# tobifinn/torch-assimilate

Measured on AMD Instinct MI355X. Metric: local analyses/sec (LETKF, 40-member), higher is better.
Workload: dtype f32

## Files before the change

### torch-assimilate_amd/csrc/letkf_tile2_kernel.h

```cpp
#pragma once
#include <type_traits>
#include "mia_common.h"
#include <hip/hip_ext.h>
#include "mia_kernels.h"
#include "mia_options.h"
#include "mia_tiles.h"
#ifdef MIA_TILE_STAMPS
namespace mia { constexpr int kT2StampN = 20, kT2StampTiles = 8192; static __device__ long long g_tile2_stamps[kT2StampTiles * kT2StampN]; }
#define MIA_TL_STAMP(i) do { if (lane == 0 && tile < mia::kT2StampTiles) mia::g_tile2_stamps[tile * mia::kT2StampN + 12 + (i)] = (long long)__builtin_amdgcn_s_memtime(); } while (0)
#endif
#include "mia_tile_localize.h"

namespace mia {

#ifdef MIA_TILE_STAMPS
#define T2_STAMP(i) do { if (lane == 0 && bid < kT2StampTiles) g_tile2_stamps[bid * kT2StampN + (i)] = (long long)__builtin_amdgcn_s_memtime(); } while (0)
#define T2_STAMP_HWID() do { if (lane == 0 && bid < kT2StampTiles) g_tile2_stamps[bid * kT2StampN + 9] = \
    (long long)(unsigned)__builtin_amdgcn_s_getreg((31 << 11) | 4) | ((long long)(unsigned)__builtin_amdgcn_s_getreg((31 << 11) | 20) << 32); } while (0)
#define T2_STAMP_REAL(i) do { if (lane == 0 && bid < kT2StampTiles) g_tile2_stamps[bid * kT2StampN + (i)] = (long long)__builtin_amdgcn_s_memrealtime(); } while (0)
#else
#define T2_STAMP(i) do { } while (0)
#define T2_STAMP_HWID() do { } while (0)
#define T2_STAMP_REAL(i) do { } while (0)
#endif

#ifndef MIA_TILE2_WAVES_UT2
#define MIA_TILE2_WAVES_UT2 4
#endif

template <int UT, int KT, bool MROWS, int LOC>
__device__ __forceinline__ void tile2_body(Tile2Params P, const Tile2Loc* loc, const int64_t bid) {
  constexpr int UMAX = 16 * UT, NB = (KT + 1) / 2, NKB = (UT + 1) / 2;
  extern __shared__ __attribute__((aligned(16))) unsigned char smem[];
  int lane = threadIdx.x, lr = lane & 15, h = lane >> 4;
  const int k = P.k, nc8 = P.nc8;
  const unsigned IMG = (unsigned)(UT * nc8) * 512u;
  unsigned char* zline = smem + IMG;
  int* ukey = reinterpret_cast<int*>(smem + IMG + 512);
  float* wdl = reinterpret_cast<float*>(ukey + UMAX);
  float* El = wdl + UMAX;

  const int64_t ntile = (P.ng + 15) >> 4;
  if (bid >= ntile) return;
  if (P.clr_counts) {
    const int ncl = *P.clr_n;
    for (int64_t i = bid * 64 + lane; i < ncl; i += ntile * 64) P.clr_counts[i] = 0;
    if (bid == 0 && lane == 0) {
      const unsigned e = *P.clr_err;
      if (e) { atomicOr(P.err_out, (int)(e << 3)); *P.clr_err = 0u; }
    }
  }
  const int64_t q8 = ntile >> 3, r8 = ntile & 7, xcd = bid & 7;
  const int64_t tile = (xcd < r8 ? xcd * (q8 + 1) : r8 * (q8 + 1) + (xcd - r8) * q8) + (bid >> 3);
  const int64_t p0 = tile << 4;
  const int npts = P.ng - p0 < 16 ? (int)(P.ng - p0) : 16;
  int64_t oc0 = P.o0 + p0;
  if (P.seg_len > 0) {
    const unsigned sgi = (unsigned)p0 / (unsigned)P.seg_len;
    oc0 = p0 - (int64_t)sgi * P.seg_len;
    P.Xa += (int64_t)sgi * P.seg_stride;
  }
  const unsigned ldxb = (unsigned)P.ldx * 4u, ldob = (unsigned)P.ldo * 4u;
  int lrc = lr < npts ? lr : npts - 1;
  bool colok = lr < npts;

#ifdef MIA_EXPERIMENTS
  const int prio_mode = (P.stagger >> 8) & 0xff, exp_trim = P.stagger >> 16;
  P.stagger &= 0xff;
  if (prio_mode == 1) __builtin_amdgcn_s_setprio(3);
  if (prio_mode >= 3) {
    const int wid = (int)(__builtin_amdgcn_s_getreg((4 << 11) | 4) & 0xf);
    const bool fast = prio_mode == 3 ? (wid & 1) : (prio_mode == 4 ? wid < 2 : (prio_mode == 5 ? wid == 0 : (wid % 3) == 0));
    if (fast) __builtin_amdgcn_s_setprio(3);
  }
  if (P.stagger > 0) {
    const int slot = (int)(__builtin_amdgcn_s_getreg((4 << 11) | 4) & 0xf);
    for (int i = 0; i < slot * P.stagger; ++i) __builtin_amdgcn_s_sleep(1);
  }
#endif
  T2_STAMP(0);
  T2_STAMP_HWID();
  T2_STAMP_REAL(10);
  int hdU = 0;
  int myidx[(UMAX + 63) / 64];
  f4w dreg[UT];
  if constexpr (LOC == 0) {
    const int4 hd = P.thdr[tile];
    hdU = hd.x;
#pragma unroll
    for (int r = 0; r < (UMAX + 63) / 64; ++r) {
      const int s = lane + 64 * r;
      myidx[r] = s < UMAX ? t2_ld<int32_t>(P.tidx + tile * UMAX, (unsigned)s * 4u) : -1;
    }
#pragma unroll
    for (int t = 0; t < UT; ++t) dreg[t] = t2_ld<f4w>(P.tD + (tile * UT + t) * 64, (unsigned)lane * 16u);
  } else {
    const TileLocOut lo = tile_localize<true, (LOC > 3 ? LOC - 4 : LOC), MIA_TAPER_GC, (LOC > 3)>(loc->scan, P.g0, P.ng, UT, tile, smem, lane);
    const TileLocLds LL(smem);
    hdU = lo.overflow ? -1 : lo.U;
    int mu[(UMAX + 63) / 64], du[UT][4];
#pragma unroll
    for (int r = 0; r < (UMAX + 63) / 64; ++r) {
      const int s = lane + 64 * r;
      mu[r] = LL.uinv[s < UMAX ? s : 0];
      mu[r] = (s < UMAX && !lo.overflow && mu[r] >= 0) ? mu[r] : kTlUmax;
    }
#pragma unroll
    for (int t = 0; t < UT; ++t)
#pragma unroll
      for (int qq = 0; qq < 4; ++qq) {
        du[t][qq] = LL.uinv[16 * t + 4 * h + qq];
        du[t][qq] = (!lo.overflow && du[t][qq] >= 0) ? du[t][qq] * 16 + lr : LL.zrow_off + lr;
      }
#pragma unroll
    for (int r = 0; r < (UMAX + 63) / 64; ++r) myidx[r] = LL.ukey[mu[r]];
#pragma unroll
    for (int t = 0; t < UT; ++t) {
      f4w v;
#pragma unroll
      for (int qq = 0; qq < 4; ++qq) v[qq] = LL.Wt[du[t][qq]];
      dreg[t] = v;
    }
    if (lane == 0) {
      if (lo.longest > loc->longest_bound) atomicMax(&loc->stats[0], lo.longest);
      else if ((tile & 63) == 0 && lo.longest > __hip_atomic_load(&loc->stats[0], __ATOMIC_RELAXED, __HIP_MEMORY_SCOPE_AGENT))
        atomicMax(&loc->stats[0], lo.longest);
      if (tile == 0) atomicOr(&loc->stats[3], kStepSampledLongest);
      if (lo.overflow) atomicAdd(&loc->stats[1], 1);
      if (lo.box_overflow) atomicOr(&loc->stats[1], MIA_TILE_BOX_OVERFLOW);
    }
    MIA_T2_SYNC();
  }
  int sg = 2 * (h & 1) + (h >> 1);
  auto load_xs = [&](int mi, float (&xr)[NB][8]) {
    const float* xbase = P.X + (int64_t)mi * k * P.ldx + P.g0 + p0;
#pragma unroll
    for (int b = 0; b < NB; ++b) {
      const int m0 = 8 * (4 * b + sg);
      if (b < NB - 1 || (k & 7) == 0) {
        const unsigned vo = (unsigned)(m0 < k ? m0 : 0) * ldxb + (unsigned)lrc * 4u;
#pragma unroll
        for (int i = 0; i < 8; ++i) xr[b][i] = t2_ld<float>(xbase, vo + (unsigned)i * ldxb);
      } else {
#pragma unroll
        for (int i = 0; i < 8; ++i) {
          const int mem = m0 + i;
          xr[b][i] = t2_ld<float>(xbase, (unsigned)(mem < k ? mem : k - 1) * ldxb + (unsigned)lrc * 4u);
        }
      }
    }
  };
  float xsb[NB][8];
  load_xs(0, xsb);
#pragma unroll
  for (int r = 0; r < (UMAX + 63) / 64; ++r) {
    const int s = lane + 64 * r;
    if (s < UMAX) ukey[s] = myidx[r];
  }
  for (int i = lane; i < 32; i += 64) reinterpret_cast<f4w*>(zline)[i] = f4w{0.f, 0.f, 0.f, 0.f};
  MIA_T2_SYNC();
  const int U = __builtin_amdgcn_readfirstlane(hdU);
  if (U < 0) {
    if (colok && h == 0) P.flags[p0 + lr] = MIA_FLAG_OVERFLOW;
    const float nanv = __builtin_nanf("");
    if (colok)
      for (int it = h; it < P.m * k; it += 4) P.Xa[(int64_t)it * P.ldo + oc0 + lr] = nanv;
    return;
  }
  T2_STAMP(1);
  {
    const int g = lane >> 4, hl = g & 1, gh = g >> 1;
    unsigned roff[UT][2];
#pragma unroll
    for (int t = 0; t < UT; ++t)
#pragma unroll
      for (int par = 0; par < 2; ++par) {
        const int idx = ukey[16 * t + ((lr - 8 * par) & 15)];
        roff[t][par] = (unsigned)(idx < 0 ? (int)P.zero_rec : idx) * (unsigned)P.rb + 16u * (unsigned)hl;
      }
    auto gather = [&](auto nc8c) {
      constexpr int NC8 = decltype(nc8c)::value;
      constexpr int NL = (UT * NC8 + 1) / 2;
#pragma unroll
      for (int u = 0; u < NL; ++u) {
        const int lA = 2 * u, lB = 2 * u + 1;
        const int tA = lA / NC8, cA = lA % NC8, tB = (lB / NC8) < UT ? lB / NC8 : UT - 1, cB = lB % NC8;
        const unsigned offA = roff[tA][cA & 1] + 32u * (unsigned)cA, offB = roff[tB][cB & 1] + 32u * (unsigned)cB;
        const unsigned off = gh ? offB : offA;
        const bool valid = 2 * u + gh < UT * NC8;
        if (valid)
          __builtin_amdgcn_global_load_lds(reinterpret_cast<const unsigned*>(P.rec + off),
                                           (__attribute__((address_space(3))) void*)(smem + u * 1024), 16, 0, 0);
      }
    };
    if (nc8 == 2 * KT - 1) gather(std::integral_constant<int, 2 * KT - 1>{});
    else gather(std::integral_constant<int, 2 * KT>{});
  }
  f2w tails[(UMAX + 63) / 64];
#pragma unroll
  for (int r = 0; r < (UMAX + 63) / 64; ++r) {
    const unsigned j = (unsigned)(myidx[r] < 0 ? (int)P.zero_rec : myidx[r]);
    tails[r] = *reinterpret_cast<const f2w*>(P.rec + (j * (unsigned)P.rb + 32u * (unsigned)nc8));
  }
  T2_STAMP(2);

  auto frag_off = [&](int t, int b) -> unsigned {
    const int c = 4 * b + sg;
    const unsigned col = (unsigned)((lr + 8 * (c & 1)) & 15) * 16u;
    return c < nc8 ? (unsigned)(t * nc8 + c) * 512u + col : IMG + col;
  };

  h8v GAh[UT][NKB], GAl[UT][NKB];
  float alpha = 0.0f;
  int deg = 0, tab_idx = 0, degmax = 0, pflag = 0;
  bool decl = false;
  auto split_x = [&](float (&xsb)[NB][8], float& xm, float& inv_sx, h8v (&xh)[NB], h8v (&xl)[NB]) {
      t2_split_x<NB, MROWS>(xsb, colok, sg, k, P.inv_k, xm, inv_sx, xh, xl);
    };
  float xm0, inv_sx0;
  f4w Z0[UT];
  {
    h8v xh[NB], xl[NB];
    split_x(xsb, xm0, inv_sx0, xh, xl);
#pragma unroll
    for (int t = 0; t < UT; ++t) Z0[t] = f4w{0.f, 0.f, 0.f, 0.f};
    f4w (&Z)[UT] = Z0;
    asm volatile("s_waitcnt vmcnt(0)" ::: "memory");
    __builtin_amdgcn_wave_barrier();
    T2_STAMP(3);
#ifdef MIA_EXPERIMENTS
    if (prio_mode == 1) __builtin_amdgcn_s_setprio(0);
    if (prio_mode == 2) __builtin_amdgcn_s_setprio(3);
#endif
    f4w G[UT][UT];
#pragma unroll
    for (int t1 = 0; t1 < UT; ++t1)
#pragma unroll
      for (int t2 = 0; t2 < UT; ++t2) G[t1][t2] = f4w{0.f, 0.f, 0.f, 0.f};
#pragma unroll
    for (int b = 0; b < NB; ++b) {
      h8v ah[UT], al[UT];
#pragma unroll
      for (int t = 0; t < UT; ++t) {
        const unsigned o = frag_off(t, b);
        ah[t] = *reinterpret_cast<const h8v*>(smem + o);
        al[t] = *reinterpret_cast<const h8v*>(smem + o + 256);
      }
#pragma unroll
      for (int t2 = 0; t2 < UT; ++t2)
#pragma unroll
        for (int t1 = 0; t1 < UT; ++t1) G[t1][t2] = t2_mfma3(G[t1][t2], ah[t1], al[t1], ah[t2], al[t2]);
#pragma unroll
      for (int t = 0; t < UT; ++t) Z[t] = t2_mfma3(Z[t], ah[t], al[t], xh[b], xl[b]);
    }
    T2_STAMP(4);
    {
      bool badrec = false;
#pragma unroll
      for (int r = 0; r < (UMAX + 63) / 64; ++r) {
        const int s = lane + 64 * r;
        if (s < UMAX) {
          wdl[s] = tails[r][0];
          El[s] = tails[r][1];
          badrec = badrec || !(tails[r][1] == tails[r][1]);
        }
      }
      if (__any(badrec)) {
        if (colok && h == 0) { P.flags[p0 + lr] = MIA_FLAG_RETRY; atomicAdd(P.retry_count, 1); }
        return;
      }
      MIA_T2_SYNC();
#pragma unroll
      for (int t = 0; t < UT; ++t) {
        const f4w e4 = *reinterpret_cast<const f4w*>(El + 16 * t + 4 * h);
        dreg[t] *= e4;
      }
    }
#pragma unroll
    for (int t = 0; t < UT; ++t)
#pragma unroll
      for (int kb = 0; kb < NKB; ++kb) {
        float gv[8];
#pragma unroll
        for (int tt = 0; tt < 2; ++tt)
#pragma unroll
          for (int q = 0; q < 4; ++q) gv[4 * tt + q] = 2 * kb + tt < UT ? G[2 * kb + tt < UT ? 2 * kb + tt : 0][t][q] * 0x1p-16f : 0.0f;
        split8(gv, GAh[t][kb], GAl[t][kb]);
      }
    f4w R[UT];
#pragma unroll
    for (int t = 0; t < UT; ++t) R[t] = f4w{0.f, 0.f, 0.f, 0.f};
    unsigned dmx = 0u;
#pragma unroll
    for (int t = 0; t < UT; ++t)
#pragma unroll
      for (int q = 0; q < 4; ++q) { const unsigned a = __float_as_uint(dreg[t][q]); dmx = a > dmx ? a : dmx; }
    dmx = t2_wave_max_u32(dmx);
    int esd;
    const float sd = pow2_scale(dmx, 0, &esd);
    const float inv_sd = __uint_as_float((unsigned)(127 - esd) << 23);
#pragma unroll
    for (int kb = 0; kb < NKB; ++kb)
      if (kb == 0 || 32 * kb < U) {
        float dv[8];
#pragma unroll
        for (int tt = 0; tt < 2; ++tt)
#pragma unroll
          for (int q = 0; q < 4; ++q) dv[4 * tt + q] = 2 * kb + tt < UT ? dreg[2 * kb + tt < UT ? 2 * kb + tt : 0][q] * sd : 0.0f;
        const h8v dh = hi8(dv);
#pragma unroll
        for (int t = 0; t < UT; ++t) {
          u4w ag = __builtin_bit_cast(u4w, GAh[t][kb]);
          ag &= 0x7fff7fffu;
          R[t] = __builtin_amdgcn_mfma_f32_16x16x32_f16(__builtin_bit_cast(h8v, ag), dh, R[t], 0, 0, 0);
        }
      }
    float L = 0.0f;
#pragma unroll
    for (int t = 0; t < UT; ++t)
#pragma unroll
      for (int q = 0; q < 4; ++q) L = __builtin_fmaxf(L, dreg[t][q] * R[t][q]);
    L = __uint_as_float(t2_max_h(__float_as_uint(L))) * inv_sd;
    L = fmaxf(L, 1e-37f) * 1.002f;
    if (!(L == L) || !(fabsf(L) < 1e30f)) { pflag |= MIA_FLAG_NONFINITE; L = 1.0f; }
    tab_idx = (int)ceilf(float(kTabPerOctave) * (__builtin_amdgcn_logf(L * P.inv_reg) + 16.0f)) + kTabIdx0;
    tab_idx = tab_idx < 0 ? 0 : (tab_idx > kTabN - 1 ? kTabN - 1 : tab_idx);
    const int2 th = t2_ld<int2>(P.tab_hdr, (unsigned)tab_idx * 8u);
    deg = th.x;
#ifdef MIA_EXPERIMENTS
    deg = deg - exp_trim > 3 ? deg - exp_trim : (deg < 3 ? deg : 3);
#endif
    alpha = __builtin_ldexpf(__int_as_float(th.y) * P.inv_reg, 16);
    decl = colok && (deg > P.dmax || deg > kTabDeg - 1);
    if (decl && h == 0) {
      P.flags[p0 + lr] = MIA_FLAG_RETRY;
      atomicAdd(P.retry_count, 1);
    }
    degmax = (int)wave_max_nonneg_dpp((colok && !decl) ? float(deg) : 0.0f);
  }
  auto row_tail = [&](const int mi, f4w (&Z)[UT], const float xm, const float inv_sx) {
    T2_STAMP(5);
    const unsigned cbase = (unsigned)tab_idx * (unsigned)(kTabDeg * 8);
    auto coef = [&](int j) -> float2 {
      return t2_ld<float2>(P.tab_c, cbase + (unsigned)(j < kTabDeg ? j : kTabDeg - 1) * 8u);
    };
    const float2 c0 = coef(0), c1 = coef(1);
    float2 cn0 = coef(2), cn1 = coef(3);
    f4w va[UT], vb[UT], aphi[UT], apsi[UT], ad2[UT];
    float inv_s2;
    {
      float zmaxf = 0.0f;
#pragma unroll
      for (int t = 0; t < UT; ++t) {
        const f4w d2 = dreg[t] * dreg[t];
        ad2[t] = alpha * d2;
        va[t] = Z[t] * d2;
#pragma unroll
        for (int q = 0; q < 4; ++q) zmaxf = __builtin_fmaxf(zmaxf, __builtin_fabsf(va[t][q]));
      }
      const unsigned zmax = t2_max_h(__float_as_uint(zmaxf));
      int es2;
      const float s2 = pow2_scale(zmax, 8, &es2);
      inv_s2 = __uint_as_float((unsigned)(127 - es2) << 23);
#pragma unroll
      for (int t = 0; t < UT; ++t) va[t] *= s2;
    }
    auto rhs_split = [&](const f4w (&tv)[UT], int kb, h8v& bh, h8v& bl) {
      float bv[8];
#pragma unroll
      for (int tt = 0; tt < 2; ++tt)
#pragma unroll
        for (int q = 0; q < 4; ++q) {
          const int tk = 2 * kb + tt < UT ? 2 * kb + tt : 0;
          bv[4 * tt + q] = 2 * kb + tt < UT ? tv[tk][q] : 0.0f;
        }
      split8(bv, bh, bl);
    };
    f4w y[UT];
    auto product = [&](const f4w (&tv)[UT]) {
      {
        h8v bh, bl;
        rhs_split(tv, 0, bh, bl);
#pragma unroll
        for (int t = 0; t < UT; ++t) y[t] = t2_mfma3(f4w{0.f, 0.f, 0.f, 0.f}, GAh[t][0], GAl[t][0], bh, bl);
      }
#pragma unroll
      for (int kb = 1; kb < NKB; ++kb)
        if (32 * kb < U) {
          h8v bh, bl;
          rhs_split(tv, kb, bh, bl);
#pragma unroll
          for (int t = 0; t < UT; ++t) y[t] = t2_mfma3(y[t], GAh[t][kb], GAl[t][kb], bh, bl);
        }
    };
    auto advance = [&](f4w (&vold)[UT], const f4w (&vcur)[UT], const float2 cj) {
      product(vcur);
#pragma unroll
      for (int t = 0; t < UT; ++t)
#pragma unroll
        for (int q = 0; q < 4; ++q) {
          const float tq = __builtin_fmaf(ad2[t][q], y[t][q], -vcur[t][q]);
          const float vn = __builtin_fmaf(2.0f, tq, -vold[t][q]);
          vold[t][q] = vn;
          aphi[t][q] = __builtin_fmaf(cj.x, vn, aphi[t][q]);
          apsi[t][q] = __builtin_fmaf(cj.y, vn, apsi[t][q]);
        }
    };
    product(va);
#pragma unroll
    for (int t = 0; t < UT; ++t)
#pragma unroll
      for (int q = 0; q < 4; ++q) {
        const float vq = __builtin_fmaf(ad2[t][q], y[t][q], -va[t][q]);
        vb[t][q] = vq;
        aphi[t][q] = __builtin_fmaf(c1.x, vq, c0.x * va[t][q]);
        apsi[t][q] = __builtin_fmaf(c1.y, vq, c0.y * va[t][q]);
      }
    int j = 2;
    for (; j + 1 <= degmax; j += 2) {
      const float2 cj = cn0, cj1 = cn1;
      cn0 = coef(j + 2); cn1 = coef(j + 3);
      advance(va, vb, cj);
      advance(vb, va, cj1);
    }
    if (j <= degmax) advance(va, vb, cn0);
    T2_STAMP(6);
    const float funs = inv_s2 * inv_sx;
    f4w xre[KT];
    {
      const float* xbase = P.X + (int64_t)mi * k * P.ldx + P.g0 + p0;
      const unsigned xo0 = (unsigned)(4 * h) * ldxb + (unsigned)lrc * 4u;
      const unsigned xolast = (unsigned)(k - 1) * ldxb + (unsigned)lrc * 4u;
#pragma unroll
      for (int tj = 0; tj < KT; ++tj)
#pragma unroll
        for (int q = 0; q < 4; ++q) {
          unsigned o = xo0 + (unsigned)(16 * tj + q) * ldxb;
          if (tj == KT - 1) o = o < xolast ? o : xolast;
          xre[tj][q] = t2_ld<float>(xbase, o);
        }
    }
    float zu = 0.0f;
#pragma unroll
    for (int t = 0; t < UT; ++t) {
      const f4w w4 = *reinterpret_cast<const f4w*>(wdl + 16 * t + 4 * h);
#pragma unroll
      for (int q = 0; q < 4; ++q) zu = fmaf(w4[q], apsi[t][q], zu);
    }
    zu = t2_add_h(zu) * (P.cs_psi * funs);
    const float mterm = xm + zu;
    h8v ph_[NKB], pl_[NKB];
#pragma unroll
    for (int kb = 0; kb < NKB; ++kb) rhs_split(aphi, kb, ph_[kb], pl_[kb]);
    const float fo = P.cs_phi * funs;
    const int tq = (lane & 15) >> 2, tp = lane & 3;
    f4w acc[KT];
    unsigned amax = 0u;
#pragma unroll
    for (int tj = 0; tj < KT; ++tj) {
      acc[tj] = f4w{0.f, 0.f, 0.f, 0.f};
      const int c = 2 * tj + (tp >> 1);
#pragma unroll
      for (int kb = 0; kb < NKB; ++kb)
        if (32 * kb < U) {
          s4v a4[2][2];
#pragma unroll
          for (int tt = 0; tt < 2; ++tt) {
            const int tb = 2 * kb + tt < UT ? 2 * kb + tt : 0;
            const unsigned col = (unsigned)((4 * h + tq + 8 * (c & 1)) & 15) * 16u + 8u * (unsigned)(tp & 1);
            const unsigned o = (c < nc8 && 2 * kb + tt < UT) ? (unsigned)(tb * nc8 + c) * 512u + col : IMG + col;
            a4[tt][0] = t2_tr_read(smem + o);
            a4[tt][1] = t2_tr_read(smem + o + 256);
          }
          typedef short s8v __attribute__((__vector_size__(8 * sizeof(short))));
          const s8v ahs = __builtin_shufflevector(a4[0][0], a4[1][0], 0, 1, 2, 3, 4, 5, 6, 7);
          const s8v als = __builtin_shufflevector(a4[0][1], a4[1][1], 0, 1, 2, 3, 4, 5, 6, 7);
          acc[tj] = t2_mfma3(acc[tj], __builtin_bit_cast(h8v, ahs), __builtin_bit_cast(h8v, als), ph_[kb], pl_[kb]);
        }
#pragma unroll
      for (int q = 0; q < 4; ++q) {
        acc[tj][q] = acc[tj][q] * fo + (mterm + P.f0 * (xre[tj][q] - xm));
        const unsigned ab = __float_as_uint(acc[tj][q]) & 0x7fffffffu;
        amax = ab > amax ? ab : amax;
      }
    }
    if (amax > 0x7149f2cau) pflag |= MIA_FLAG_NONFINITE;
    if (colok && !decl) {
      float* obase = P.Xa + (int64_t)mi * k * P.ldo + oc0;
      const unsigned olane = (unsigned)(4 * h) * ldob + (unsigned)lr * 4u;
#pragma unroll
      for (int tj = 0; tj < KT; ++tj)
#pragma unroll
        for (int q = 0; q < 4; ++q)
          if (tj < KT - 1 || 16 * tj + 4 * h + q < k)
            *reinterpret_cast<float*>(reinterpret_cast<char*>(obase) + (olane + (unsigned)(16 * tj + q) * ldob)) = acc[tj][q];
    } else {
      pflag = 0;
    }
  };
  row_tail(0, Z0, xm0, inv_sx0);
  if constexpr (MROWS) {
    for (int mi = 1; mi < P.m; ++mi) {
      asm volatile("" : "+v"(lane), "+v"(lr), "+v"(h));
      lrc = lr < npts ? lr : npts - 1;
      colok = lr < npts;
      sg = 2 * (h & 1) + (h >> 1);
      load_xs(mi, xsb);
      float xm, inv_sx;
      h8v xh[NB], xl[NB];
      split_x(xsb, xm, inv_sx, xh, xl);
      f4w Z[UT];
#pragma unroll
      for (int t = 0; t < UT; ++t) Z[t] = f4w{0.f, 0.f, 0.f, 0.f};
#pragma unroll
      for (int b = 0; b < NB; ++b) {
#pragma unroll
        for (int t = 0; t < UT; ++t) {
          const unsigned o = frag_off(t, b);
          const h8v ah = *reinterpret_cast<const h8v*>(smem + o), al = *reinterpret_cast<const h8v*>(smem + o + 256);
          Z[t] = t2_mfma3(Z[t], ah, al, xh[b], xl[b]);
        }
      }
      row_tail(mi, Z, xm, inv_sx);
    }
  }
  T2_STAMP(7);
  {
    const unsigned long long fb = __ballot(pflag != 0);
    const bool anyf = ((fb >> lr) & 0x0001000100010001ull) != 0ull;
    if (h == 0 && colok && !decl) P.flags[p0 + lr] = (anyf ? MIA_FLAG_NONFINITE : 0) | (deg << 8);
    if constexpr (LOC > 0) {
      if (fb != 0ull && lane == 0) atomicOr(&loc->stats[3], kStepNonfinite);
    }
  }
  T2_STAMP(8);
  T2_STAMP_REAL(11);
}


}
```

### torch-assimilate_amd/csrc/mia_tiles.h

```cpp
#pragma once
#include "mia_common.h"

namespace mia {

constexpr int kTileSlack = 8;

static inline int tile_ut_for(int p_max) {
  const int ut = (p_max + kTileSlack + 15) >> 4;
  return ut < 1 ? 1 : ut;
}

struct TileListLayout { size_t hdr, idx, D, bytes; int ut; int64_t ntile; };
static inline TileListLayout tile_list_layout(int64_t ng, int ut) {
  TileListLayout L;
  L.ut = ut;
  L.ntile = (ng + 15) >> 4;
  size_t o = 0;
  L.hdr = o; o = align_up(o + (size_t)(L.ntile > 0 ? L.ntile : 1) * 16, 256);
  L.idx = o; o = align_up(o + (size_t)(L.ntile > 0 ? L.ntile : 1) * 16 * ut * sizeof(int32_t), 256);
  L.D = o; o = align_up(o + (size_t)(L.ntile > 0 ? L.ntile : 1) * ut * 1024, 256);
  L.bytes = o;
  return L;
}

static inline int split_nc8(int k) { return (k + 7) >> 3; }
static inline int split_rec_bytes(int k) { return 32 * split_nc8(k) + 16; }

__device__ __forceinline__ float pow2_scale(unsigned magbits, int target, int* es_out) {
  const int e = (int)(magbits >> 23) - 127;
  int es = (magbits >> 23) == 0u ? 0 : target - e;
  es = es < -60 ? -60 : (es > 60 ? 60 : es);
  *es_out = es;
  return __uint_as_float((unsigned)(127 + es) << 23);
}

using h8v = __attribute__((ext_vector_type(8))) _Float16;
using h2v = __attribute__((ext_vector_type(2))) _Float16;
using f2w = __attribute__((ext_vector_type(2))) float;
using f4w = __attribute__((ext_vector_type(4))) float;
using u4w = __attribute__((ext_vector_type(4))) unsigned;

__device__ __forceinline__ void split8(const float (&x)[8], h8v& hi, h8v& lo) {
  u4w hu, lu;
#pragma unroll
  for (int i = 0; i < 4; ++i) {
    const f2w v = {x[2 * i], x[2 * i + 1]};
    const h2v a = __builtin_convertvector(v, h2v);
    hu[i] = __builtin_bit_cast(unsigned, a);
  }
  asm("s_nop 2\n\t"
      "v_fma_mixlo_f16 %0, %4, -1.0, %8 op_sel:[0,0,0] op_sel_hi:[1,0,0]\n\t"
      "v_fma_mixhi_f16 %0, %4, -1.0, %9 op_sel:[1,0,0] op_sel_hi:[1,0,0]\n\t"
      "v_fma_mixlo_f16 %1, %5, -1.0, %10 op_sel:[0,0,0] op_sel_hi:[1,0,0]\n\t"
      "v_fma_mixhi_f16 %1, %5, -1.0, %11 op_sel:[1,0,0] op_sel_hi:[1,0,0]\n\t"
      "v_fma_mixlo_f16 %2, %6, -1.0, %12 op_sel:[0,0,0] op_sel_hi:[1,0,0]\n\t"
      "v_fma_mixhi_f16 %2, %6, -1.0, %13 op_sel:[1,0,0] op_sel_hi:[1,0,0]\n\t"
      "v_fma_mixlo_f16 %3, %7, -1.0, %14 op_sel:[0,0,0] op_sel_hi:[1,0,0]\n\t"
      "v_fma_mixhi_f16 %3, %7, -1.0, %15 op_sel:[1,0,0] op_sel_hi:[1,0,0]\n\t"
      "s_nop 1"
      : "=&v"(lu[0]), "=&v"(lu[1]), "=&v"(lu[2]), "=&v"(lu[3])
      : "v"(hu[0]), "v"(hu[1]), "v"(hu[2]), "v"(hu[3]), "v"(x[0]), "v"(x[1]), "v"(x[2]), "v"(x[3]), "v"(x[4]), "v"(x[5]),
        "v"(x[6]), "v"(x[7]));
  hi = __builtin_bit_cast(h8v, hu);
  lo = __builtin_bit_cast(h8v, lu);
}
__device__ __forceinline__ void split8_tied(const float (&x)[8], h8v& hi, h8v& lo) {
  u4w hu, lu;
#pragma unroll
  for (int i = 0; i < 4; ++i) {
    const f2w v = {x[2 * i], x[2 * i + 1]};
    const h2v a = __builtin_convertvector(v, h2v);
    hu[i] = __builtin_bit_cast(unsigned, a);
    lu[i] = hu[i];
  }
  asm("v_fma_mixlo_f16 %0, %0, -1.0, %4 op_sel:[0,0,0] op_sel_hi:[1,0,0]\n\t"
      "v_fma_mixhi_f16 %0, %0, -1.0, %5 op_sel:[1,0,0] op_sel_hi:[1,0,0]\n\t"
      "v_fma_mixlo_f16 %1, %1, -1.0, %6 op_sel:[0,0,0] op_sel_hi:[1,0,0]\n\t"
      "v_fma_mixhi_f16 %1, %1, -1.0, %7 op_sel:[1,0,0] op_sel_hi:[1,0,0]\n\t"
      "v_fma_mixlo_f16 %2, %2, -1.0, %8 op_sel:[0,0,0] op_sel_hi:[1,0,0]\n\t"
      "v_fma_mixhi_f16 %2, %2, -1.0, %9 op_sel:[1,0,0] op_sel_hi:[1,0,0]\n\t"
      "v_fma_mixlo_f16 %3, %3, -1.0, %10 op_sel:[0,0,0] op_sel_hi:[1,0,0]\n\t"
      "v_fma_mixhi_f16 %3, %3, -1.0, %11 op_sel:[1,0,0] op_sel_hi:[1,0,0]\n\t"
      "s_nop 1"
      : "+v"(lu[0]), "+v"(lu[1]), "+v"(lu[2]), "+v"(lu[3])
      : "v"(x[0]), "v"(x[1]), "v"(x[2]), "v"(x[3]), "v"(x[4]), "v"(x[5]), "v"(x[6]), "v"(x[7]));
  hi = __builtin_bit_cast(h8v, hu);
  lo = __builtin_bit_cast(h8v, lu);
}
__device__ __forceinline__ void split8n(const float (&x)[8], h8v& hi, h8v& lo) {
  u4w hu, lu;
  asm("s_nop 3\n\t"
      "v_cvt_pk_f16_f32 %0, -%8, -%9\n\t"
      "v_cvt_pk_f16_f32 %1, -%10, -%11\n\t"
      "v_cvt_pk_f16_f32 %2, -%12, -%13\n\t"
      "v_cvt_pk_f16_f32 %3, -%14, -%15\n\t"
      "v_fma_mixlo_f16 %4, %0, -1.0, -%8 op_sel:[0,0,0] op_sel_hi:[1,0,0]\n\t"
      "v_fma_mixhi_f16 %4, %0, -1.0, -%9 op_sel:[1,0,0] op_sel_hi:[1,0,0]\n\t"
      "v_fma_mixlo_f16 %5, %1, -1.0, -%10 op_sel:[0,0,0] op_sel_hi:[1,0,0]\n\t"
      "v_fma_mixhi_f16 %5, %1, -1.0, -%11 op_sel:[1,0,0] op_sel_hi:[1,0,0]\n\t"
      "v_fma_mixlo_f16 %6, %2, -1.0, -%12 op_sel:[0,0,0] op_sel_hi:[1,0,0]\n\t"
      "v_fma_mixhi_f16 %6, %2, -1.0, -%13 op_sel:[1,0,0] op_sel_hi:[1,0,0]\n\t"
      "v_fma_mixlo_f16 %7, %3, -1.0, -%14 op_sel:[0,0,0] op_sel_hi:[1,0,0]\n\t"
      "v_fma_mixhi_f16 %7, %3, -1.0, -%15 op_sel:[1,0,0] op_sel_hi:[1,0,0]\n\t"
      "s_nop 1"
      : "=&v"(hu[0]), "=&v"(hu[1]), "=&v"(hu[2]), "=&v"(hu[3]), "=&v"(lu[0]), "=&v"(lu[1]), "=&v"(lu[2]), "=&v"(lu[3])
      : "v"(x[0]), "v"(x[1]), "v"(x[2]), "v"(x[3]), "v"(x[4]), "v"(x[5]), "v"(x[6]), "v"(x[7]));
  hi = __builtin_bit_cast(h8v, hu);
  lo = __builtin_bit_cast(h8v, lu);
}
__device__ __forceinline__ h8v hi8(const float (&x)[8]) {
  h8v hi;
#pragma unroll
  for (int i = 0; i < 4; ++i) {
    const f2w v = {x[2 * i], x[2 * i + 1]};
    const h2v a = __builtin_convertvector(v, h2v);
    hi[2 * i] = a[0]; hi[2 * i + 1] = a[1];
  }
  return hi;
}

#define MIA_T2_SYNC() do { asm volatile("s_waitcnt lgkmcnt(0)" ::: "memory"); __builtin_amdgcn_wave_barrier(); } while (0)
__device__ __forceinline__ float t2_add_h(float v) {
  typedef unsigned u2v __attribute__((ext_vector_type(2)));
  u2v r = __builtin_amdgcn_permlane32_swap(__float_as_uint(v), __float_as_uint(v), false, false);
  v = __uint_as_float(r.x) + __uint_as_float(r.y);
  r = __builtin_amdgcn_permlane16_swap(__float_as_uint(v), __float_as_uint(v), false, false);
  return __uint_as_float(r.x) + __uint_as_float(r.y);
}
__device__ __forceinline__ unsigned t2_max_h(unsigned u) {
  typedef unsigned u2v __attribute__((ext_vector_type(2)));
  u2v r = __builtin_amdgcn_permlane32_swap(u, u, false, false);
  u = r.x > r.y ? r.x : r.y;
  r = __builtin_amdgcn_permlane16_swap(u, u, false, false);
  return r.x > r.y ? r.x : r.y;
}
template <int NB, bool TIED>
__device__ __forceinline__ void t2_split_x(float (&xsb)[NB][8], const bool colok, const int sg, const int k, const float inv_k,
                                           float& xm, float& inv_sx, h8v (&xh)[NB], h8v (&xl)[NB]) {
#pragma clang fp contract(off)
  float xs = 0.0f;
  unsigned xmax = 0u;
  if ((k & 7) == 0) {
    float lm[NB];
#pragma unroll
    for (int b = 0; b < NB; ++b) lm[b] = (colok && 8 * (4 * b + sg) < k) ? 1.0f : 0.0f;
#pragma unroll
    for (int b = 0; b < NB; ++b)
#pragma unroll
      for (int i = 0; i < 8; ++i) xs = __builtin_fmaf(xsb[b][i], lm[b], xs);
    xm = t2_add_h(xs) * inv_k;
    float xmaxf = 0.0f;
#pragma unroll
    for (int b = 0; b < NB; ++b) {
      const float xml = xm * lm[b];
#pragma unroll
      for (int i = 0; i < 8; ++i) {
        xsb[b][i] = __builtin_fmaf(xsb[b][i], lm[b], -xml);
        xmaxf = __builtin_fmaxf(xmaxf, __builtin_fabsf(xsb[b][i]));
      }
    }
    xmax = __float_as_uint(xmaxf);
  } else {
#pragma unroll
    for (int b = 0; b < NB; ++b)
#pragma unroll
      for (int i = 0; i < 8; ++i) {
        const bool live = colok && 8 * (4 * b + sg) + i < k;
        xsb[b][i] = live ? xsb[b][i] : 0.0f;
        xs += xsb[b][i];
      }
    xm = t2_add_h(xs) * inv_k;
#pragma unroll
    for (int b = 0; b < NB; ++b)
#pragma unroll
      for (int i = 0; i < 8; ++i) {
        const bool live = colok && 8 * (4 * b + sg) + i < k;
        xsb[b][i] = live ? xsb[b][i] - xm : 0.0f;
        const unsigned a = __float_as_uint(xsb[b][i]) & 0x7fffffffu;
        xmax = a > xmax ? a : xmax;
      }
  }
  xmax = t2_max_h(xmax);
  int esx;
  const float sx = pow2_scale(xmax, 9, &esx);
  inv_sx = __uint_as_float((unsigned)(127 - esx) << 23);
#pragma unroll
  for (int b = 0; b < NB; ++b) {
    float t8[8];
#pragma unroll
    for (int i = 0; i < 8; ++i) t8[i] = xsb[b][i] * sx;
    if constexpr (TIED) split8_tied(t8, xh[b], xl[b]);
    else split8(t8, xh[b], xl[b]);
  }
}
__device__ __forceinline__ unsigned t2_wave_max_u32(unsigned u) {
  unsigned t;
  t = (unsigned)__builtin_amdgcn_update_dpp(0, (int)u, 0xB1, 0xf, 0xf, false); u = u > t ? u : t;
  t = (unsigned)__builtin_amdgcn_update_dpp(0, (int)u, 0x4E, 0xf, 0xf, false); u = u > t ? u : t;
  t = (unsigned)__builtin_amdgcn_update_dpp(0, (int)u, 0x124, 0xf, 0xf, false); u = u > t ? u : t;
  t = (unsigned)__builtin_amdgcn_update_dpp(0, (int)u, 0x128, 0xf, 0xf, false); u = u > t ? u : t;
  const unsigned a = (unsigned)__builtin_amdgcn_readlane((int)u, 0), b = (unsigned)__builtin_amdgcn_readlane((int)u, 16);
  const unsigned c = (unsigned)__builtin_amdgcn_readlane((int)u, 32), d = (unsigned)__builtin_amdgcn_readlane((int)u, 48);
  const unsigned ab = a > b ? a : b, cd = c > d ? c : d;
  return ab > cd ? ab : cd;
}
__device__ __forceinline__ f4w t2_mfma3(f4w acc, const h8v ah, const h8v al, const h8v bh, const h8v bl) {
  acc = __builtin_amdgcn_mfma_f32_16x16x32_f16(al, bh, acc, 0, 0, 0);
  acc = __builtin_amdgcn_mfma_f32_16x16x32_f16(ah, bl, acc, 0, 0, 0);
  return __builtin_amdgcn_mfma_f32_16x16x32_f16(ah, bh, acc, 0, 0, 0);
}
template <typename T>
__device__ __forceinline__ T t2_ld(const void* base, unsigned byte_off) {
  return *reinterpret_cast<const T*>(reinterpret_cast<const char*>(base) + byte_off);
}
typedef short s4v __attribute__((__vector_size__(4 * sizeof(short))));
__device__ __forceinline__ s4v t2_tr_read(const unsigned char* lds_addr) {
  return __builtin_amdgcn_ds_read_tr16_b64_v4i16((__attribute__((address_space(3))) s4v*)lds_addr);
}


struct SplitPackJob { const float* Yb; const float* d; unsigned char* rec; int k; };

__device__ inline void pack_split_wave(const SplitPackJob& J, int64_t P, int64_t block, float* lds) {
  const int lane = threadIdx.x & 63;
  const int k = J.k, nc8 = (k + 7) >> 3, rb = 32 * nc8 + 16;
  const int ls = (k + 1) | 1;
  float* scl = lds + 64 * ls;
  const int64_t j0 = block * 64;
  const int64_t j = j0 + lane;
  const bool real = j < P;
  const int64_t jc = real ? j : (P > 0 ? P - 1 : 0);
  const float dj = (real && P > 0) ? J.d[jc] : 0.0f;
  constexpr int kRowsInFlight = 40;
  for (int i0 = 0; i0 < k; i0 += kRowsInFlight) {
    float v[kRowsInFlight];
#pragma unroll
    for (int u = 0; u < kRowsInFlight; ++u) {
      const int i = i0 + u < k ? i0 + u : k - 1;
      v[u] = (P > 0) ? J.Yb[(int64_t)i * P + jc] : 0.0f;
    }
#pragma unroll
    for (int u = 0; u < kRowsInFlight; ++u)
      if (i0 + u < k) lds[lane * ls + i0 + u] = real ? v[u] : 0.0f;
  }
  do { asm volatile("s_waitcnt lgkmcnt(0)" ::: "memory"); __builtin_amdgcn_wave_barrier(); } while (0);
  unsigned mx = 0u;
  for (int i = 0; i < k; ++i) {
    const unsigned a = __float_as_uint(lds[lane * ls + i]) & 0x7fffffffu;
    mx = a > mx ? a : mx;
  }
  int es;
  const float sc = pow2_scale(mx, 9, &es);
  const float wd = dj * sc;
  const bool bad = mx >= 0x7f800000u || !(fabsf(wd) < 3.0e38f);
  scl[lane] = sc;
  if (j <= P) {
    const float E = bad ? __builtin_nanf("") : __uint_as_float((unsigned)(127 - es) << 23);
    *reinterpret_cast<f4w*>(J.rec + j * rb + 32 * nc8) = f4w{wd, E, 0.0f, 0.0f};
  }
  do { asm volatile("s_waitcnt lgkmcnt(0)" ::: "memory"); __builtin_amdgcn_wave_barrier(); } while (0);
  const int nvalid = P + 1 - j0 < 64 ? (int)(P + 1 - j0) : 64;
  const int nq = nvalid * nc8;
  int r = lane / nc8, c = lane - r * nc8;
  const int dr = 64 / nc8, dc = 64 - dr * nc8;
  for (int q = lane; q < nq; q += 64) {
    const float s = scl[r];
    float x[8];
#pragma unroll
    for (int i = 0; i < 8; ++i) x[i] = 8 * c + i < k ? lds[r * ls + 8 * c + i] * s : 0.0f;
    h8v hi, lo;
    split8(x, hi, lo);
    unsigned char* o = J.rec + (j0 + r) * rb + 32 * c;
    *reinterpret_cast<h8v*>(o) = hi;
    *reinterpret_cast<h8v*>(o + 16) = lo;
    r += dr; c += dc;
    if (c >= nc8) { c -= nc8; ++r; }
  }
}

static inline size_t split_pack_lds(int k) { return ((size_t)64 * ((k + 1) | 1) + 64) * sizeof(float); }

__device__ __forceinline__ void pack_split_lean_request(const SplitPackJob& J, int64_t P, int64_t block, float* lds) {
  const int lane = threadIdx.x & 63;
  const int64_t j = block * 64 + lane;
  const int64_t jc = j < P ? j : (P > 0 ? P - 1 : 0);
  if (P > 0)
    for (int i = 0; i < J.k; ++i)
      __builtin_amdgcn_global_load_lds(reinterpret_cast<const unsigned*>(J.Yb + (int64_t)i * P + jc),
                                       (__attribute__((address_space(3))) void*)(lds + i * 64), 4, 0, 0);
}
__device__ __forceinline__ void pack_split_lean_finish(const SplitPackJob& J, int64_t P, int64_t block, const float* lds) {
  const int lane = threadIdx.x & 63;
  const int k = J.k, nc8 = (k + 7) >> 3, rb = 32 * nc8 + 16;
  const int64_t j = block * 64 + lane;
  const bool real = j < P;
  const float dj = (real && P > 0) ? J.d[j] : 0.0f;
  asm volatile("s_waitcnt vmcnt(0)" ::: "memory");
  __builtin_amdgcn_wave_barrier();
  unsigned mx = 0u;
  if (real)
    for (int i = 0; i < k; ++i) {
      const unsigned a = __float_as_uint(lds[i * 64 + lane]) & 0x7fffffffu;
      mx = a > mx ? a : mx;
    }
  int es;
  const float sc = pow2_scale(mx, 9, &es);
  const float wd = dj * sc;
  const bool bad = mx >= 0x7f800000u || !(fabsf(wd) < 3.0e38f);
  if (j > P) return;
  unsigned char* o = J.rec + j * rb;
  const float E = bad ? __builtin_nanf("") : __uint_as_float((unsigned)(127 - es) << 23);
  *reinterpret_cast<f4w*>(o + 32 * nc8) = f4w{wd, E, 0.0f, 0.0f};
  for (int c = 0; c < nc8; ++c) {
    float x[8];
#pragma unroll
    for (int i = 0; i < 8; ++i) x[i] = (real && 8 * c + i < k) ? lds[(8 * c + i) * 64 + lane] * sc : 0.0f;
    h8v hi, lo;
    split8(x, hi, lo);
    *reinterpret_cast<h8v*>(o + 32 * c) = hi;
    *reinterpret_cast<h8v*>(o + 32 * c + 16) = lo;
  }
}
static inline size_t split_pack_lean_lds(int k) { return (size_t)64 * k * sizeof(float); }

struct ScanParams;
int split_pack_launch(const float* Yb, const float* d, int k, int64_t P, void* rec, hipStream_t stream);
int tile_lists_launch(const double* grid_xyz, int64_t g0, int64_t ng, int64_t P, int n_coord, const int32_t* coord_group,
                      const double* gc_c, int n_r, double gc_eps, int taper, int ut, void* tile_lists, int32_t* stats,
                      void* index_ws, hipStream_t stream, const SplitPackJob* pack, bool bucket = false, const int* counts = nullptr,
                      const double* period = nullptr);
struct Tile2Params {
  const float* X; int64_t ldx; int m, k;
  int64_t g0, ng;
  const unsigned char* rec; int rb, nc8; int64_t zero_rec;
  const int4* thdr; const int32_t* tidx; const f4w* tD;
  float inv_reg, f0, inv_k, cs_phi, cs_psi;
  float* Xa; int64_t ldo, o0; int32_t* flags; int32_t* retry_count;
  int dmax;
  const int2* tab_hdr; const float2* tab_c;
  int seg_len; int64_t seg_stride;
  int* clr_counts; const int* clr_n; unsigned* clr_err; int32_t* err_out;
  int stagger;
};
struct Tile2Housekeeping { int* counts; const int* n; unsigned* err; int32_t* err_out; };
bool tile2_covers(int m, int k, int p_max, int extra_blocks, int64_t ldx, int64_t ldo, int64_t ng);
bool tile2_records_addressable(int k, int64_t P);
int tile2_analysis_launch(const float* X, int64_t ldx, int m, int k, int64_t g0, int64_t ng, const void* rec, int64_t P,
                          const void* tile_lists, int ut, float inf_factor, float* Xa, int64_t ldo, int64_t o0,
                          int32_t* flags, int32_t* retry_count, int dmax, const int2* tab_hdr, const float2* tab_c,
                          hipStream_t stream, int seg_len = 0, int64_t seg_stride = 0, const Tile2Housekeeping* hk = nullptr,
                          const struct Tile2Loc* loc = nullptr);
bool tile2f_covers(int m, int k, int ut, int n_coord);
int tile2f_launch(const Tile2Params& tp, const struct Tile2Loc& loc, int ut, int kt, hipStream_t stream);
size_t tile2_lds_bytes(int ut, int k);

int tile2p_launch_any(const Tile2Params& tp, int ut, int kt, hipStream_t stream);
bool lketkf_tile_covers(int m, int k, int p_max, int extra_blocks, int64_t ldx, int64_t ldo, int64_t ng, int64_t P);
int lketkf_tile_launch(const float* X, int64_t ldx, int m, int k, int64_t g0, int64_t ng, const float* Yb, const float* d,
                       int64_t P, const void* tile_lists, int ut, float inf_factor, float gamma, float* Xa, int64_t ldo,
                       int64_t o0, int32_t* flags, int32_t* retry_count, int dmax, const int2* tab_hdr, const float2* tab_c,
                       hipStream_t stream, int seg_len = 0, int64_t seg_stride = 0, const Tile2Housekeeping* hk = nullptr);

}
```

Measured before the change: 2.591 billion.

## Fold psi weight row into spare GA matrix row to drop apsi accumulators

When the tile has an unused row (U < UMAX), the scaled localisation weight vector is embedded into the last row of the G operator. The psi reduction then falls out of the existing MFMA products, read from one output element, instead of keeping a second per-lane apsi polynomial accumulator and doing a final dot product. This removes one FMA stream and a vector of registers per Chebyshev step. Coefficient loads are also repacked so that one unaligned float2 load fetches the psi coefficient of step j and the phi coefficient of step j+1. The cost is an extra scaling pass, a closing MFMA for the last psi term, and a fallback path that keeps the old dot-product accumulation when no spare row exists.

```diff
diff --git a/torch-assimilate_amd/csrc/letkf_tile2_kernel.h b/torch-assimilate_amd/csrc/letkf_tile2_kernel.h
--- a/torch-assimilate_amd/csrc/letkf_tile2_kernel.h
+++ b/torch-assimilate_amd/csrc/letkf_tile2_kernel.h
@@ -211,6 +211,8 @@
   };
 
   h8v GAh[UT][NKB], GAl[UT][NKB];
+  bool spare = false;
+  float inv_sw = 1.0f;
   float alpha = 0.0f;
   int deg = 0, tab_idx = 0, degmax = 0, pflag = 0;
   bool decl = false;
@@ -276,6 +278,28 @@
         dreg[t] *= e4;
       }
     }
+    f4w wrow[UT];
+    {
+      static_assert(UMAX <= 128, "the zero line stands in for wdl");
+      const float* wsrc = (U < UMAX && lr == 15 ? wdl : reinterpret_cast<const float*>(zline)) + 4 * h;
+      float wmaxf = 0.0f;
+#pragma unroll
+      for (int t = 0; t < UT; ++t) {
+        wrow[t] = *reinterpret_cast<const f4w*>(wsrc + 16 * t);
+#pragma unroll
+        for (int q = 0; q < 4; ++q) wmaxf = __builtin_fmaxf(wmaxf, __builtin_fabsf(wrow[t][q]));
+      }
+      const unsigned wmx = (unsigned)__builtin_amdgcn_readlane((int)t2_max_h(__float_as_uint(wmaxf)), 15);
+      int esw;
+      const float sw = pow2_scale(wmx, 14, &esw);
+      spare = U < UMAX && esw > -60 && esw < 60;
+      inv_sw = __uint_as_float((unsigned)(127 - esw) << 23);
+      const float swm = spare ? sw : 0.0f;
+#pragma unroll
+      for (int t = 0; t < UT; ++t)
+#pragma unroll
+        for (int q = 0; q < 4; ++q) asm("v_mul_legacy_f32 %0, %0, %1" : "+v"(wrow[t][q]) : "v"(swm));
+    }
 #pragma unroll
     for (int t = 0; t < UT; ++t)
 #pragma unroll
@@ -284,7 +308,12 @@
 #pragma unroll
         for (int tt = 0; tt < 2; ++tt)
 #pragma unroll
-          for (int q = 0; q < 4; ++q) gv[4 * tt + q] = 2 * kb + tt < UT ? G[2 * kb + tt < UT ? 2 * kb + tt : 0][t][q] * 0x1p-16f : 0.0f;
+          for (int q = 0; q < 4; ++q) {
+            const int tk = 2 * kb + tt < UT ? 2 * kb + tt : 0;
+            if (2 * kb + tt >= UT) gv[4 * tt + q] = 0.0f;
+            else if (t == UT - 1) gv[4 * tt + q] = __builtin_fmaf(G[tk][t][q], 0x1p-16f, wrow[tk][q]);
+            else gv[4 * tt + q] = G[tk][t][q] * 0x1p-16f;
+          }
         split8(gv, GAh[t][kb], GAl[t][kb]);
       }
     f4w R[UT];
@@ -341,12 +370,15 @@
   auto row_tail = [&](const int mi, f4w (&Z)[UT], const float xm, const float inv_sx) {
     T2_STAMP(5);
     const unsigned cbase = (unsigned)tab_idx * (unsigned)(kTabDeg * 8);
-    auto coef = [&](int j) -> float2 {
-      return t2_ld<float2>(P.tab_c, cbase + (unsigned)(j < kTabDeg ? j : kTabDeg - 1) * 8u);
-    };
-    const float2 c0 = coef(0), c1 = coef(1);
-    float2 cn0 = coef(2), cn1 = coef(3);
-    f4w va[UT], vb[UT], aphi[UT], apsi[UT], ad2[UT];
+    typedef float f2a4 __attribute__((ext_vector_type(2), aligned(4)));
+    auto coef = [&](int j, int back) -> float2 {
+      const f2a4 c = t2_ld<f2a4>(reinterpret_cast<const char*>(P.tab_c) - back, cbase + (unsigned)(j < kTabDeg ? j : kTabDeg - 1) * 8u);
+      return float2{c[0], c[1]};
+    };
+    const float2 c0 = coef(0, 0), c1 = coef(1, 0);
+    float2 cn0 = coef(2, 4), cn1 = coef(3, 4);
+    const float cpl = t2_ld<float>(P.tab_c, cbase + (unsigned)(degmax > 1 ? degmax : 1) * 8u + 4u);
+    f4w va[UT], vb[UT], aphi[UT], ad2[UT];
     float inv_s2;
     {
       float zmaxf = 0.0f;
@@ -393,8 +425,33 @@
           for (int t = 0; t < UT; ++t) y[t] = t2_mfma3(y[t], GAh[t][kb], GAl[t][kb], bh, bl);
         }
     };
+    product(va);
+    float zrow = 0.0f, zdot = 0.0f;
+    auto psi_dot = [&](const f4w (&tv)[UT], const float cpsi) {
+      if (!spare) {
+        float d = 0.0f;
+#pragma unroll
+        for (int t = 0; t < UT; ++t) {
+          const f4w w4 = *reinterpret_cast<const f4w*>(wdl + 16 * t + 4 * h);
+#pragma unroll
+          for (int q = 0; q < 4; ++q) d = __builtin_fmaf(w4[q], tv[t][q], d);
+        }
+        zdot = __builtin_fmaf(cpsi, d, zdot);
+      }
+    };
+    zrow = c0.y * y[UT - 1][3];
+#pragma unroll
+    for (int t = 0; t < UT; ++t)
+#pragma unroll
+      for (int q = 0; q < 4; ++q) {
+        const float vq = __builtin_fmaf(ad2[t][q], y[t][q], -va[t][q]);
+        vb[t][q] = vq;
+        aphi[t][q] = __builtin_fmaf(c1.x, vq, c0.x * va[t][q]);
+      }
+    psi_dot(va, c0.y);
     auto advance = [&](f4w (&vold)[UT], const f4w (&vcur)[UT], const float2 cj) {
       product(vcur);
+      zrow = __builtin_fmaf(cj.x, y[UT - 1][3], zrow);
 #pragma unroll
       for (int t = 0; t < UT; ++t)
 #pragma unroll
@@ -402,28 +459,38 @@
           const float tq = __builtin_fmaf(ad2[t][q], y[t][q], -vcur[t][q]);
           const float vn = __builtin_fmaf(2.0f, tq, -vold[t][q]);
           vold[t][q] = vn;
-          aphi[t][q] = __builtin_fmaf(cj.x, vn, aphi[t][q]);
-          apsi[t][q] = __builtin_fmaf(cj.y, vn, apsi[t][q]);
-        }
-    };
-    product(va);
-#pragma unroll
-    for (int t = 0; t < UT; ++t)
-#pragma unroll
-      for (int q = 0; q < 4; ++q) {
-        const float vq = __builtin_fmaf(ad2[t][q], y[t][q], -va[t][q]);
-        vb[t][q] = vq;
-        aphi[t][q] = __builtin_fmaf(c1.x, vq, c0.x * va[t][q]);
-        apsi[t][q] = __builtin_fmaf(c1.y, vq, c0.y * va[t][q]);
-      }
+          aphi[t][q] = __builtin_fmaf(cj.y, vn, aphi[t][q]);
+        }
+      asm volatile("" : "+v"(zrow));
+#pragma unroll
+      for (int t = 0; t < UT; ++t) asm volatile("" : "+v"(aphi[t][0]), "+v"(aphi[t][1]), "+v"(aphi[t][2]), "+v"(aphi[t][3]));
+      psi_dot(vcur, cj.x);
+    };
+    auto close = [&](const f4w (&tv)[UT], const float cpsi) {
+      psi_dot(tv, cpsi);
+      if (spare) {
+        f4w yc = f4w{0.f, 0.f, 0.f, 0.f};
+#pragma unroll
+        for (int kb = 0; kb < NKB; ++kb)
+          if (kb == 0 || 32 * kb < U) {
+            h8v bh, bl;
+            rhs_split(tv, kb, bh, bl);
+            yc = t2_mfma3(yc, GAh[UT - 1][kb], GAl[UT - 1][kb], bh, bl);
+          }
+        zrow = __builtin_fmaf(cpsi, yc[3], zrow);
+      }
+    };
     int j = 2;
     for (; j + 1 <= degmax; j += 2) {
-      const float2 cj = cn0, cj1 = cn1;
-      cn0 = coef(j + 2); cn1 = coef(j + 3);
-      advance(va, vb, cj);
-      advance(vb, va, cj1);
-    }
-    if (j <= degmax) advance(va, vb, cn0);
+      const int jn = j + 2 < kTabDeg - 1 ? j + 2 : kTabDeg - 2;
+      advance(va, vb, cn0);
+      cn0 = coef(jn, 4);
+      advance(vb, va, cn1);
+      cn1 = coef(jn, -4);
+    }
+    if (j <= degmax) { advance(va, vb, cn0); close(va, cpl); }
+    else close(vb, cpl);
+    const float zu0 = spare ? t2_bcast_h3(zrow) * inv_sw : t2_add_h(zdot);
     T2_STAMP(6);
     const float funs = inv_s2 * inv_sx;
     f4w xre[KT];
@@ -440,14 +507,7 @@
           xre[tj][q] = t2_ld<float>(xbase, o);
         }
     }
-    float zu = 0.0f;
-#pragma unroll
-    for (int t = 0; t < UT; ++t) {
-      const f4w w4 = *reinterpret_cast<const f4w*>(wdl + 16 * t + 4 * h);
-#pragma unroll
-      for (int q = 0; q < 4; ++q) zu = fmaf(w4[q], apsi[t][q], zu);
-    }
-    zu = t2_add_h(zu) * (P.cs_psi * funs);
+    const float zu = zu0 * (P.cs_psi * funs);
     const float mterm = xm + zu;
     h8v ph_[NKB], pl_[NKB];
 #pragma unroll
diff --git a/torch-assimilate_amd/csrc/mia_tiles.h b/torch-assimilate_amd/csrc/mia_tiles.h
--- a/torch-assimilate_amd/csrc/mia_tiles.h
+++ b/torch-assimilate_amd/csrc/mia_tiles.h
@@ -133,6 +133,12 @@
   u = r.x > r.y ? r.x : r.y;
   r = __builtin_amdgcn_permlane16_swap(u, u, false, false);
   return r.x > r.y ? r.x : r.y;
+}
+__device__ __forceinline__ float t2_bcast_h3(float v) {
+  typedef unsigned u2v __attribute__((ext_vector_type(2)));
+  u2v r = __builtin_amdgcn_permlane32_swap(__float_as_uint(v), __float_as_uint(v), false, false);
+  r = __builtin_amdgcn_permlane16_swap(r.y, r.y, false, false);
+  return __uint_as_float(r.y);
 }
 template <int NB, bool TIED>
 __device__ __forceinline__ void t2_split_x(float (&xsb)[NB][8], const bool colok, const int sg, const int k, const float inv_k,
```

Result: slower. 2.565 billion (-1.0%).
